# mauro3/KissMCMC.jl

Hardware: NVIDIA B200
Metric: walker_steps_per_s (higher is better)
Workload: dtype f64

## Files before the change

### kissmcmc.jl_b200/csrc/kmc_device.cuh

```cuda
#pragma once
#include <cstdint>
#ifndef KMC_U48_BITS
#define KMC_U48_BITS 0
#endif
#include <cuda_runtime.h>

namespace kmc {

__device__ __forceinline__ double dmul(double a, double b) { return __dmul_rn(a, b); }
__device__ __forceinline__ double dadd(double a, double b) { return __dadd_rn(a, b); }
__device__ __forceinline__ double dsub(double a, double b) { return __dsub_rn(a, b); }
__device__ __forceinline__ double ddiv(double a, double b) { return __ddiv_rn(a, b); }

__device__ __forceinline__ void split3_pair(double v0, double v1, unsigned (&pk)[3]) {
    float f0 = __double2float_rn(v0), f1 = __double2float_rn(v1);
#pragma unroll
    for (int pc = 0; pc < 3; ++pc) {
        unsigned u;
        asm("cvt.rn.bf16x2.f32 %0, %1, %2;" : "=r"(u) : "f"(f1), "f"(f0));
        pk[pc] = u;
        if (pc < 2) {
            f0 = __fsub_rn(f0, __uint_as_float(u << 16));
            f1 = __fsub_rn(f1, __uint_as_float(u & 0xFFFF0000u));
        }
    }
}

struct Philox4 {
    uint32_t r0, r1, r2, r3;
};

struct PhiloxKeys {
    uint32_t k0[10], k1[10];
};

__host__ __device__ inline PhiloxKeys philox_keys(uint64_t seed) {
    PhiloxKeys ks;
    uint32_t a = (uint32_t)seed, b = (uint32_t)(seed >> 32);
    for (int r = 0; r < 10; ++r) {
        ks.k0[r] = a;
        ks.k1[r] = b;
        a += 0x9E3779B9u;
        b += 0xBB67AE85u;
    }
    return ks;
}

__device__ __forceinline__ void mul_wide(uint32_t a, uint32_t b, uint32_t &hi, uint32_t &lo) {
    asm("{\n\t.reg .u64 t;\n\tmul.wide.u32 t, %2, %3;\n\tmov.b64 {%1, %0}, t;\n\t}" : "=r"(hi), "=r"(lo) : "r"(a), "r"(b));
}

__device__ __forceinline__ Philox4 philox4x32_10(uint32_t c0, uint32_t c1, uint32_t c2, uint32_t c3,
                                                 const PhiloxKeys &ks) {
#pragma unroll
    for (int r = 0; r < 10; ++r) {
        uint32_t hi0, lo0, hi1, lo1;
        mul_wide(0xD2511F53u, c0, hi0, lo0);
        mul_wide(0xCD9E8D57u, c2, hi1, lo1);
        c0 = hi1 ^ c1 ^ ks.k0[r];
        c1 = lo1;
        c2 = hi0 ^ c3 ^ ks.k1[r];
        c3 = lo0;
    }
    return Philox4{c0, c1, c2, c3};
}

__device__ __forceinline__ uint32_t lemire_retry(const PhiloxKeys &ks, uint32_t walker, uint32_t iter_lo,
                                              uint32_t iter_hi, uint32_t batch, uint32_t nhalf, uint32_t lemire_t) {
    uint32_t hi, lo, attempt = 0;
    do {
        ++attempt;
        const Philox4 rr = philox4x32_10(walker, iter_lo, iter_hi, batch | (attempt << 8), ks);
        mul_wide(rr.r0, nhalf, hi, lo);
    } while (lo < lemire_t);
    return hi;
}

__device__ __forceinline__ void draw(const PhiloxKeys &ks, uint32_t walker, uint32_t iter_lo, uint32_t iter_hi,
                                     uint32_t batch, uint32_t nhalf, uint32_t lemire_t, uint32_t &partner_local,
                                     double &uz, double &uacc) {
    const Philox4 r = philox4x32_10(walker, iter_lo, iter_hi, batch, ks);
    uint32_t hi, lo;
    mul_wide(r.r0, nhalf, hi, lo);
    if (lo < lemire_t)
        hi = lemire_retry(ks, walker, iter_lo, iter_hi, batch, nhalf, lemire_t);
    partner_local = hi;
    const uint64_t bz = ((uint64_t)r.r1 << 16) | (r.r2 >> 16);
    const uint64_t ba = ((uint64_t)(r.r2 & 0xFFFFu) << 32) | r.r3;
#if KMC_U48_BITS
    uz = __dadd_rn(__longlong_as_double((long long)(0x3FF0000000000000ULL | (bz << 4))), -1.0);
    uacc = __dadd_rn(__longlong_as_double((long long)(0x3FF0000000000000ULL | (ba << 4))), -1.0);
#else
    uz = (double)bz * 0x1p-48;
    uacc = (double)ba * 0x1p-48;
#endif
}

__device__ __forceinline__ Philox4 philox_normals(const PhiloxKeys &ks, uint32_t c0, uint32_t c1, uint32_t c2, uint32_t c3,
                                                  double &z0, double &z1) {
    const Philox4 r = philox4x32_10(c0, c1, c2, c3, ks);
    const double u1 = ((double)r.r0 + 1.0) * 0x1p-32;
    const double u2 = (double)r.r1 * 0x1p-32;
    const double rad = sqrt(-2.0 * log(u1));
    double sn, cs;
    sincospi(2.0 * u2, &sn, &cs);
    z0 = rad * cs;
    z1 = rad * sn;
    return r;
}


constexpr int KIND_EXPONENTIAL = 0;
constexpr int KIND_ROSENBROCK = 1;
constexpr int KIND_GAUSSIAN = 2;
constexpr int KIND_LOGNORMAL = 3;
constexpr int KIND_LOGISTIC = 4;

template <int D>
struct Exponential {
    static constexpr int kind = KIND_EXPONENTIAL;
    static constexpr int nparams = 0;
    double unused;
    __device__ __forceinline__ double logpdf(const double (&x)[D]) const {
        double s = x[0];
        bool neg = x[0] < 0.0;
#pragma unroll
        for (int c = 1; c < D; ++c) {
            neg = neg || (x[c] < 0.0);
            s = dadd(s, x[c]);
        }
        return neg ? -CUDART_INF : -s;
    }
};

__device__ __forceinline__ double ddiv_by(double a, double b, double y) {
    const double aa = fabs(a);
    if (y != 0.0 && aa > 0x1p-900 && aa < 0x1p900) {
        const double q0 = a * y;
        const double r0 = fma(-b, q0, a);
        const double q1 = fma(r0, y, q0);
        const double r1 = fma(-b, q1, a);
        return fma(r1, y, q1);
    }
    return __ddiv_rn(a, b);
}

template <int D>
struct Rosenbrock {
    static_assert(D == 2, "rosenbrock is 2-D");
    static constexpr int kind = KIND_ROSENBROCK;
    static constexpr int nparams = 3;
    double p[4];
    __device__ __forceinline__ double logpdf(const double (&x)[D]) const {
        const double t = dsub(x[1], dmul(x[0], x[0]));
        const double q = dmul(p[1], dmul(t, t));
        const double m = dsub(p[0], x[0]);
        const double r = dadd(q, dmul(m, m));
        return ddiv_by(-r, p[2], p[3]);
    }
};

template <int D>
struct Gaussian {
    static constexpr int kind = KIND_GAUSSIAN;
    static constexpr int nparams = D + D * D + 1;
    double p[D + D * D + 1];
    __device__ __forceinline__ double logpdf(const double (&x)[D]) const {
        double c[D];
#pragma unroll
        for (int j = 0; j < D; ++j) c[j] = dsub(x[j], p[j]);
        double ss = 0.0;
#pragma unroll
        for (int i = 0; i < D; ++i) {
            double y = 0.0;
#pragma unroll
            for (int j = 0; j < D; ++j) y = dadd(y, dmul(p[D + i * D + j], c[j]));
            ss = dadd(ss, dmul(y, y));
        }
        return dsub(p[D + D * D], dmul(0.5, ss));
    }
};

template <int D>
struct LogNormal {
    static_assert(D == 1, "lognormal is 1-D");
    static constexpr int kind = KIND_LOGNORMAL;
    static constexpr int nparams = 3;
    double p[3];
    __device__ __forceinline__ double logpdf(const double (&x)[D]) const {
        if (!(x[0] > 0.0)) return (x[0] != x[0]) ? x[0] : -CUDART_INF;
        const double lx = log(x[0]);
        const double t = ddiv(dsub(lx, p[0]), p[1]);
        return dsub(dsub(-lx, dmul(0.5, dmul(t, t))), p[2]);
    }
};

template <int D>
__device__ __forceinline__ void load_row(const double *__restrict__ p, double (&v)[D]) {
    if constexpr (D % 2 == 0) {
#pragma unroll
        for (int c = 0; c < D; c += 2) {
            const double2 t = *reinterpret_cast<const double2 *>(p + c);
            v[c] = t.x;
            v[c + 1] = t.y;
        }
    } else {
#pragma unroll
        for (int c = 0; c < D; ++c) v[c] = p[c];
    }
}

template <int D>
__device__ __forceinline__ void load_row_cg(const double *p, double (&v)[D]) {
    if constexpr (D % 2 == 0) {
#pragma unroll
        for (int c = 0; c < D; c += 2) {
            const double2 t = __ldcg(reinterpret_cast<const double2 *>(p + c));
            v[c] = t.x;
            v[c + 1] = t.y;
        }
    } else {
#pragma unroll
        for (int c = 0; c < D; ++c) v[c] = __ldcg(p + c);
    }
}

template <int D>
__device__ __forceinline__ void store_row(double *p, const double (&v)[D]) {
    if constexpr (D % 2 == 0) {
#pragma unroll
        for (int c = 0; c < D; c += 2) *reinterpret_cast<double2 *>(p + c) = make_double2(v[c], v[c + 1]);
    } else {
#pragma unroll
        for (int c = 0; c < D; ++c) p[c] = v[c];
    }
}

template <int D>
__device__ __forceinline__ void store_row_cs(double *p, const double (&v)[D]) {
    if constexpr (D % 2 == 0) {
#pragma unroll
        for (int c = 0; c < D; c += 2) __stcs(reinterpret_cast<double2 *>(p + c), make_double2(v[c], v[c + 1]));
    } else {
#pragma unroll
        for (int c = 0; c < D; ++c) __stcs(p + c, v[c]);
    }
}

}
```

### kissmcmc.jl_b200/csrc/kmc_kernels.cuh

```cuda
#pragma once
#include <math_constants.h>
#include <type_traits>

#include "kmc_device.cuh"

namespace kmc {

template <int D>
__host__ __device__ constexpr int max_threads() { return D <= 4 ? 448 : 256; }
template <int D>
__host__ __device__ constexpr int min_blocks() { return D <= 4 ? 2 : 1; }
template <int D>
__host__ __device__ constexpr int in_flight() { return D <= 2 ? 2 : (D <= 8 ? 2 : 1); }

struct RunParams {
    double *x;
    double *lp;
    unsigned *nacc;
    double *chain_x;
    double *chain_lp;
    const long long *rp_partner;
    const double *rp_z;
    const double *rp_u;
    long long rp_t0;
    long long nw;
    unsigned nhalf;
    unsigned per_cta;
    unsigned shard_begin, shard_end;
    long long chain_nw;
    long long h0, h1;
    long long n0;
    long long phase0;
    long long sidx0;
    long long nthin, ns;
    double sia, span, nm1;
    float nm1f, margin;
    PhiloxKeys keys;
    unsigned id_base[2];
    unsigned lemire_t;
    unsigned long long *barrier;
    unsigned long long bar_base;
    const double *peer_x[8];
    unsigned long long *peer_flags[8];
    int npeers, rank;
    unsigned long long epoch_base;
};

__device__ __forceinline__ void barrier_arrive(unsigned long long *ctr) {
    asm volatile("red.release.gpu.global.add.u64 [%0], 1;" ::"l"(ctr) : "memory");
}
__device__ __forceinline__ void barrier_wait(const unsigned long long *ctr, unsigned long long target) {
    unsigned long long v;
    long long t0 = 0;
    unsigned spins = 0;
    do {
        asm volatile("ld.relaxed.gpu.global.u64 %0, [%1];" : "=l"(v) : "l"(ctr) : "memory");
        if (v < target && (++spins & 0xFFFu) == 0) {
            if (t0 == 0) t0 = clock64();
            else if (clock64() - t0 > 40000000000LL) __trap();
        }
    } while (v < target);
    asm volatile("fence.acq_rel.gpu;" ::: "memory");
}

__device__ __forceinline__ void barrier_wait_acquire(const unsigned long long *ctr, unsigned long long target) {
    unsigned long long v;
    long long t0 = 0;
    unsigned spins = 0;
    do {
        asm volatile("ld.acquire.gpu.global.u64 %0, [%1];" : "=l"(v) : "l"(ctr) : "memory");
        if (v < target && (++spins & 0xFFFu) == 0) {
            if (t0 == 0) t0 = clock64();
            else if (clock64() - t0 > 40000000000LL) __trap();
        }
    } while (v < target);
}

template <bool SKIP_LOGZ>
__device__ __forceinline__ bool accept_exact(double nm1, double z, double p1, double p0, double u) {
    double lhs;
    if constexpr (SKIP_LOGZ) lhs = dsub(p1, p0);
    else lhs = dsub(dadd(dmul(nm1, log(z)), p1), p0);
    return lhs >= log(u);
}

__device__ __forceinline__ float lg2_approx(float v) {
    float r;
    asm("lg2.approx.ftz.f32 %0, %1;" : "=f"(r) : "f"(v));
    return r;
}

template <bool REPLAY>
__device__ __forceinline__ float filter_q(const RunParams &p, double z, double u) {
    const float zf = (float)z, uf = (float)u;
    bool ok = uf > 1e-30f;
    if constexpr (REPLAY) ok = ok && uf < 1e30f;
    ok = ok && zf > 0.0625f && zf < 16.0f;
    const float q = fmaf(p.nm1f, lg2_approx(zf), -lg2_approx(uf));
    return ok ? q : CUDART_NAN_F;
}

template <bool REPLAY>
__device__ __forceinline__ void step_draws(const RunParams &p, long long h, unsigned i, unsigned &j, double &z,
                                           double &u) {
    if constexpr (REPLAY) {
        const long long slot = (h - 2 * p.rp_t0) * (long long)p.nhalf + i;
        j = (unsigned)__ldcs(p.rp_partner + slot);
        z = __ldcs(p.rp_z + slot);
        u = __ldcs(p.rp_u + slot);
    } else {
        const unsigned long long t = (unsigned long long)(h >> 1);
        const unsigned batch = (unsigned)(h & 1);
        unsigned pl;
        double uz;
        draw(p.keys, p.id_base[batch] + i, (unsigned)t, (unsigned)(t >> 32), batch, p.nhalf, p.lemire_t, pl, uz, u);
        j = (batch ? 0u : p.nhalf) + pl;
        const double s = dadd(dmul(uz, p.span), p.sia);
        z = dmul(s, s);
    }
}

template <bool REPLAY, bool SKIP_LOGZ>
__device__ __forceinline__ bool accept_slow(const RunParams &p, long long h, unsigned i, double z, double p1, double p0) {
    unsigned j;
    double z2, u;
    step_draws<REPLAY>(p, h, i, j, z2, u);
    return accept_exact<SKIP_LOGZ>(p.nm1, z, p1, p0, u);
}

struct DrawRec {
    unsigned j;
    float q;
    double z;
};

__device__ __forceinline__ size_t chain_row(const RunParams &p, long long sidx, unsigned batch, unsigned i) {
    return (size_t)sidx * p.chain_nw + (batch ? (size_t)(p.shard_end - p.shard_begin) : 0) + (i - p.shard_begin);
}

template <int D>
__device__ __forceinline__ void chain_store(const RunParams &p, size_t o, bool acc, const double (&y)[D],
                                            const double (&xk)[D], double p1, double lpk) {
    if (acc) store_row_cs<D>(p.chain_x + o * D, y);
    else store_row_cs<D>(p.chain_x + o * D, xk);
    __stcs(p.chain_lp + o, acc ? p1 : lpk);
}

template <int D>
__device__ __forceinline__ void load_row_sys(const double *p, double (&v)[D]) {
    if constexpr (D % 2 == 0) {
#pragma unroll
        for (int c = 0; c < D; c += 2)
            asm volatile("ld.relaxed.sys.global.v2.f64 {%0, %1}, [%2];" : "=d"(v[c]), "=d"(v[c + 1]) : "l"(p + c) : "memory");
    } else {
#pragma unroll
        for (int c = 0; c < D; ++c) asm volatile("ld.relaxed.sys.global.f64 %0, [%1];" : "=d"(v[c]) : "l"(p + c) : "memory");
    }
}

__device__ __forceinline__ void bulk_row_g2s(void *smem_dst, const void *gsrc, unsigned bytes, unsigned long long *bar) {
    asm volatile("cp.async.bulk.shared::cluster.global.mbarrier::complete_tx::bytes [%0], [%1], %2, [%3];" ::"r"(
                     (unsigned)__cvta_generic_to_shared(smem_dst)),
                 "l"(gsrc), "r"(bytes), "r"((unsigned)__cvta_generic_to_shared(bar))
                 : "memory");
}
__device__ __forceinline__ void kbar_init(unsigned long long *bar, unsigned count) {
    asm volatile("mbarrier.init.shared::cta.b64 [%0], %1;" ::"r"((unsigned)__cvta_generic_to_shared(bar)), "r"(count));
    asm volatile("fence.mbarrier_init.release.cluster;" ::: "memory");
}
__device__ __forceinline__ void kbar_expect_tx(unsigned long long *bar, unsigned bytes) {
    asm volatile("mbarrier.arrive.expect_tx.shared::cta.b64 _, [%0], %1;" ::"r"((unsigned)__cvta_generic_to_shared(bar)),
                 "r"(bytes)
                 : "memory");
}
__device__ __forceinline__ void kbar_wait(unsigned long long *bar, unsigned parity) {
    const unsigned a = (unsigned)__cvta_generic_to_shared(bar);
    const long long t0 = clock64();
    unsigned done = 0;
    while (!done) {
        asm volatile(
            "{\n\t.reg .pred p;\n\t"
            "mbarrier.try_wait.parity.shared::cta.b64 p, [%1], %2;\n\t"
            "selp.u32 %0, 1, 0, p;\n\t}"
            : "=r"(done)
            : "r"(a), "r"(parity)
            : "memory");
        if (!done && clock64() - t0 > 20000000000LL) __trap();
    }
}

__device__ __forceinline__ void cross_gpu_barrier(const RunParams &p, unsigned long long epoch) {
    if ((int)threadIdx.x < p.npeers) {
        unsigned long long *dst = p.peer_flags[threadIdx.x] + p.rank;
        asm volatile("fence.acq_rel.sys;" ::: "memory");
        asm volatile("st.release.sys.global.u64 [%0], %1;" ::"l"(dst), "l"(epoch) : "memory");
        const unsigned long long *mine = p.peer_flags[p.rank] + threadIdx.x;
        const long long t0 = clock64();
        unsigned long long v;
        do {
            asm volatile("ld.acquire.sys.global.u64 %0, [%1];" : "=l"(v) : "l"(mine) : "memory");
            if (v < epoch && clock64() - t0 > 20000000000LL) __trap();
        } while (v < epoch);
    }
}

template <template <int> class Dn, int D, bool REPLAY, bool PEER = false>
static __global__ void __launch_bounds__(max_threads<D>(), min_blocks<D>()) emcee_run_kernel(const RunParams p,
                                                                                    const Dn<D> dn) {
    constexpr int U = in_flight<D>();
    const unsigned shard_size = p.shard_end - p.shard_begin;
    constexpr bool BULK = PEER && (D % 2 == 0);
    __shared__ __align__(16) double prow[BULK ? U * max_threads<D>() * D : 1];
    __shared__ unsigned long long pbar;
    unsigned pphase = 0;
    if constexpr (BULK) {
        if (threadIdx.x == 0) kbar_init(&pbar, 1);
        __syncthreads();
    }
    const unsigned tid = threadIdx.x, nthr = blockDim.x;
    const unsigned base = p.shard_begin + blockIdx.x * p.per_cta;
    const unsigned cnt = base >= p.shard_end ? 0u : min(p.per_cta, p.shard_end - base);

    DrawRec dr[U];
    auto make_draws = [&](long long h, unsigned l, DrawRec &r) {
        unsigned j;
        double z, u;
        step_draws<REPLAY>(p, h, base + l, j, z, u);
        r.j = j;
        r.z = z;
        r.q = filter_q<REPLAY>(p, z, u);
    };
#pragma unroll
    for (int q = 0; q < U; ++q) {
        const unsigned l = tid + q * nthr;
        if (l < cnt) make_draws(p.h0, l, dr[q]);
    }

    long long n = p.n0, phase = p.phase0, sidx = p.sidx0;
    unsigned long long target = p.bar_base;
    for (long long h = p.h0; h < p.h1; ++h) {
        const int batch = (int)(h & 1);
        const bool store = (n > 0) && (phase == 0);
        const unsigned a0 = batch ? p.nhalf : 0u;

        for (unsigned g = 0; g * nthr < cnt; g += U) {
            if (g > 0) {
#pragma unroll
                for (int q = 0; q < U; ++q) {
                    const unsigned l = tid + (g + q) * nthr;
                    if (l < cnt) make_draws(h, l, dr[q]);
                }
            }
            double xj[U][D], xk[U][D], lpk[U];
            if constexpr (BULK) {
                if (tid == 0) {
                    unsigned rows = 0;
#pragma unroll
                    for (int q = 0; q < U; ++q) {
                        const unsigned first = (g + q) * nthr;
                        rows += first < cnt ? min(nthr, cnt - first) : 0u;
                    }
                    kbar_expect_tx(&pbar, rows * D * 8);
                }
            }
#pragma unroll
            for (int q = 0; q < U; ++q) {
                const unsigned l = tid + (g + q) * nthr;
                if (l < cnt) {
                    const size_t k = (size_t)a0 + base + l;
                    if constexpr (PEER) {
                        const unsigned pos = dr[q].j >= p.nhalf ? dr[q].j - p.nhalf : dr[q].j;
                        const double *src = p.peer_x[pos / shard_size] + (size_t)dr[q].j * D;
                        if constexpr (BULK) bulk_row_g2s(prow + ((size_t)q * nthr + tid) * D, src, D * 8, &pbar);
                        else load_row_sys<D>(src, xj[q]);
                    } else {
                        load_row_cg<D>(p.x + (size_t)dr[q].j * D, xj[q]);
                    }
                    load_row<D>(p.x + k * D, xk[q]);
                    lpk[q] = p.lp[k];
                }
            }
            if constexpr (BULK) {
                kbar_wait(&pbar, pphase);
                pphase ^= 1;
#pragma unroll
                for (int q = 0; q < U; ++q) {
                    const unsigned l = tid + (g + q) * nthr;
                    if (l < cnt) {
#pragma unroll
                        for (int c = 0; c < D; ++c) xj[q][c] = prow[((size_t)q * nthr + tid) * D + c];
                    }
                }
                __syncthreads();
            }
#pragma unroll
            for (int q = 0; q < U; ++q) {
                const unsigned l = tid + (g + q) * nthr;
                if (l >= cnt) continue;
                const size_t k = (size_t)a0 + base + l;
                const double z = dr[q].z;
                double y[D];
#pragma unroll
                for (int c = 0; c < D; ++c) y[c] = dadd(xj[q][c], dmul(z, dsub(xk[q][c], xj[q][c])));
                const double p1 = dn.logpdf(y);
                const double tt = (p1 - lpk[q]) + (double)dr[q].q * 0.6931471805599453;
                bool acc;
                if (tt > (double)p.margin) acc = true;
                else if (tt < -(double)p.margin) acc = false;
                else acc = accept_slow<REPLAY, (D == 1 && !REPLAY)>(p, h, base + l, z, p1, lpk[q]);
                if (acc) {
                    store_row<D>(p.x + k * D, y);
                    p.lp[k] = p1;
                    p.nacc[k] += 1u;
                }
                if (store) chain_store<D>(p, chain_row(p, sidx, (unsigned)batch, base + l), acc, y, xk[q], p1, lpk[q]);
            }
        }
        if (batch == 1) {
            if (n == 0) {
                for (unsigned l = tid; l < cnt; l += nthr) {
                    p.nacc[base + l] = 0u;
                    p.nacc[(size_t)p.nhalf + base + l] = 0u;
                }
            }
            if (store) ++sidx;
            ++n;
            if (++phase == p.nthin) phase = 0;
        }
        if (h + 1 < p.h1) {
            target += gridDim.x;
            __syncthreads();
            if (gridDim.x > 1 && tid == 0) barrier_arrive(p.barrier);
#pragma unroll
            for (int q = 0; q < U; ++q) {
                const unsigned l = tid + q * nthr;
                if (l < cnt) make_draws(h + 1, l, dr[q]);
            }
            if (gridDim.x > 1) {
                if (tid == 0) barrier_wait(p.barrier, target);
                __syncthreads();
            }
            if constexpr (PEER) {
                if (blockIdx.x == 0) cross_gpu_barrier(p, p.epoch_base + (unsigned long long)(h - p.h0) + 1);
                target += gridDim.x;
                __syncthreads();
                if (gridDim.x > 1) {
                    if (tid == 0) {
                        barrier_arrive(p.barrier);
                        barrier_wait(p.barrier, target);
                    }
                    __syncthreads();
                }
            }
        }
    }
}

constexpr int kBulkThreads = 256;
#ifndef KMC_BULK_STORE_ALL
#define KMC_BULK_STORE_ALL 0
#endif
#ifndef KMC_BULK_CTAS
#define KMC_BULK_CTAS 3
#endif

__device__ __forceinline__ void bulk_s2g(void *gdst, const void *smem_src, unsigned bytes) {
    asm volatile("cp.async.bulk.global.shared::cta.bulk_group [%0], [%1], %2;" ::"l"(gdst),
                 "r"((unsigned)__cvta_generic_to_shared(smem_src)), "r"(bytes)
                 : "memory");
    asm volatile("cp.async.bulk.commit_group;" ::: "memory");
}

template <template <int> class Dn, int D, bool PEER>
static __global__ void __launch_bounds__(kBulkThreads, KMC_BULK_CTAS) emcee_bulk_kernel(const RunParams p, const Dn<D> dn) {
    static_assert(D % 2 == 0, "rows must be multiples of 16 bytes");
    extern __shared__ __align__(128) unsigned char bulk_smem[];
    constexpr unsigned T = kBulkThreads, ROWB = D * 8;
    double *xown = reinterpret_cast<double *>(bulk_smem);
    double *xpart = xown + 2 * T * D;
    unsigned long long *ldbar = reinterpret_cast<unsigned long long *>(xpart + T * D);
    const unsigned tid = threadIdx.x;
    const unsigned base = p.shard_begin + blockIdx.x * p.per_cta;
    const unsigned cnt = base >= p.shard_end ? 0u : min(p.per_cta, p.shard_end - base);
    const unsigned shard_size = p.shard_end - p.shard_begin;
    const unsigned ngroups = (cnt + T - 1) / T;
    if (tid == 0) kbar_init(ldbar, 1);
    __syncthreads();
    unsigned ldphase = 0, gcount = 0;

    DrawRec dr;
    auto make_draw = [&](long long h, unsigned l) {
        unsigned j;
        double z, u;
        step_draws<false>(p, h, base + l, j, z, u);
        dr.j = j;
        dr.z = z;
        dr.q = filter_q<false>(p, z, u);
    };
    if (tid < cnt) make_draw(p.h0, tid);

    long long n = p.n0, phase = p.phase0, sidx = p.sidx0;
    unsigned long long target = p.bar_base;
    for (long long h = p.h0; h < p.h1; ++h) {
        const unsigned batch = (unsigned)(h & 1);
        const bool store = (n > 0) && (phase == 0);
        const size_t a0 = batch ? (size_t)p.nhalf : 0;
        for (unsigned g = 0; g < ngroups; ++g, ++gcount) {
            const unsigned rows = min(T, cnt - g * T);
            const unsigned l = g * T + tid;
            const bool live = tid < rows;
            double *own = xown + (size_t)(gcount & 1) * T * D;
            if (tid == 0) asm volatile("cp.async.bulk.wait_group.read 1;" ::: "memory");
            __syncthreads();
            if (tid == 0) {
                kbar_expect_tx(ldbar, rows * ROWB * 2);
                bulk_row_g2s(own, p.x + (a0 + base + (size_t)g * T) * D, rows * ROWB, ldbar);
            }
            if (g > 0 && live) make_draw(h, l);
            if (live) {
                const unsigned pos = dr.j >= p.nhalf ? dr.j - p.nhalf : dr.j;
                const double *src = (PEER ? p.peer_x[pos / shard_size] : p.x) + (size_t)dr.j * D;
                bulk_row_g2s(xpart + (size_t)tid * D, src, ROWB, ldbar);
            }
            const size_t k = a0 + base + l;
            const double lpk = live ? p.lp[k] : 0.0;
            kbar_wait(ldbar, ldphase);
            ldphase ^= 1;
            if (live) {
                double xk[D], xj[D], y[D];
#pragma unroll
                for (int c = 0; c < D; c += 2) {
                    const double2 a2 = *reinterpret_cast<const double2 *>(own + (size_t)tid * D + c);
                    const double2 b2 = *reinterpret_cast<const double2 *>(xpart + (size_t)tid * D + c);
                    xk[c] = a2.x;
                    xk[c + 1] = a2.y;
                    xj[c] = b2.x;
                    xj[c + 1] = b2.y;
                }
                const double z = dr.z;
#pragma unroll
                for (int c = 0; c < D; ++c) y[c] = dadd(xj[c], dmul(z, dsub(xk[c], xj[c])));
                const double p1 = dn.logpdf(y);
                const double tt = (p1 - lpk) + (double)dr.q * 0.6931471805599453;
                bool acc;
                if (tt > (double)p.margin) acc = true;
                else if (tt < -(double)p.margin) acc = false;
                else acc = accept_slow<false, false>(p, h, base + l, z, p1, lpk);
                if (acc) {
#if KMC_BULK_STORE_ALL
#pragma unroll
                    for (int c = 0; c < D; c += 2)
                        *reinterpret_cast<double2 *>(own + (size_t)tid * D + c) = make_double2(y[c], y[c + 1]);
#else
                    store_row<D>(p.x + k * D, y);
#endif
                    p.lp[k] = p1;
                    p.nacc[k] += 1u;
                }
                if (store) chain_store<D>(p, chain_row(p, sidx, batch, base + l), acc, y, xk, p1, lpk);
            }
#if KMC_BULK_STORE_ALL
            asm volatile("fence.proxy.async.shared::cta;" ::: "memory");
            __syncthreads();
            if (tid == 0) bulk_s2g(p.x + (a0 + base + (size_t)g * T) * D, own, rows * ROWB);
#endif
        }
        if (batch == 1) {
            if (n == 0) {
                for (unsigned l = tid; l < cnt; l += T) {
                    p.nacc[base + l] = 0u;
                    p.nacc[(size_t)p.nhalf + base + l] = 0u;
                }
            }
            if (store) ++sidx;
            ++n;
            if (++phase == p.nthin) phase = 0;
        }
#if KMC_BULK_STORE_ALL
        if (tid == 0) {
            asm volatile("cp.async.bulk.wait_group 0;" ::: "memory");
            asm volatile("fence.proxy.async;" ::: "memory");
        }
#else
        asm volatile("fence.proxy.async;" ::: "memory");
#endif
        if (h + 1 < p.h1) {
            target += gridDim.x;
            __syncthreads();
            if (gridDim.x > 1 && tid == 0) barrier_arrive(p.barrier);
            if (tid < cnt) make_draw(h + 1, tid);
            if (gridDim.x > 1) {
                if (tid == 0) barrier_wait(p.barrier, target);
                __syncthreads();
            }
#if !KMC_BULK_STORE_ALL
            asm volatile("fence.proxy.async;" ::: "memory");
#endif
            if constexpr (PEER) {
                if (blockIdx.x == 0) cross_gpu_barrier(p, p.epoch_base + (unsigned long long)(h - p.h0) + 1);
                target += gridDim.x;
                __syncthreads();
                if (gridDim.x > 1) {
                    if (tid == 0) {
                        barrier_arrive(p.barrier);
                        barrier_wait(p.barrier, target);
                    }
                    __syncthreads();
                }
            }
        }
    }
}

#ifndef KMC_SMEM_ROUNDS
#define KMC_SMEM_ROUNDS 7
#endif
#ifndef KMC_SMEM_THREADS
#define KMC_SMEM_THREADS 256
#endif
#ifndef KMC_SMEM_CTAS
#define KMC_SMEM_CTAS 2
#endif
#ifndef KMC_SMEM_SPLIT
#define KMC_SMEM_SPLIT 4
#endif
constexpr int kRounds = KMC_SMEM_ROUNDS;
constexpr int kSmemSplit = KMC_SMEM_SPLIT;
#ifndef KMC_SMEM_AHEAD
#define KMC_SMEM_AHEAD 2
#endif
constexpr int kAhead = KMC_SMEM_AHEAD;
static_assert(kSmemSplit >= kAhead && kSmemSplit <= kRounds, "the first partner gathers need their draws");
constexpr int kSmemThreads = KMC_SMEM_THREADS;
constexpr int kSmemCtas = KMC_SMEM_CTAS;

__device__ __forceinline__ double lds_f64(unsigned a) {
    double v;
    asm volatile("ld.shared.f64 %0, [%1];" : "=d"(v) : "r"(a));
    return v;
}
__device__ __forceinline__ void sts_f64(unsigned a, double v) {
    asm volatile("st.shared.f64 [%0], %1;" ::"r"(a), "d"(v) : "memory");
}
__device__ __forceinline__ unsigned lds_u32(unsigned a) {
    unsigned v;
    asm volatile("ld.shared.u32 %0, [%1];" : "=r"(v) : "r"(a));
    return v;
}
__device__ __forceinline__ void sts_u32(unsigned a, unsigned v) {
    asm volatile("st.shared.u32 [%0], %1;" ::"r"(a), "r"(v) : "memory");
}

template <template <int> class Dn, int D, bool REPLAY>
static __global__ void __launch_bounds__(kSmemThreads, kSmemCtas) emcee_smem_kernel(const RunParams p, const Dn<D> dn) {
    extern __shared__ __align__(16) unsigned char smem_raw[];
    const unsigned nthr = blockDim.x;
    const unsigned L = 2 * p.per_cta;
    const unsigned wid = p.shard_begin + blockIdx.x * p.per_cta + threadIdx.x;
    const unsigned sbase = (unsigned)__cvta_generic_to_shared(smem_raw) + 8u * threadIdx.x;
    const unsigned nbase = (unsigned)__cvta_generic_to_shared(smem_raw) + 8u * (D + 1) * L + 4u * threadIdx.x;
    double *const grow = p.x + (size_t)wid * D;
    unsigned nv;
    {
        const unsigned base = p.shard_begin + blockIdx.x * p.per_cta;
        const unsigned cnt = base >= p.shard_end ? 0u : min(p.per_cta, p.shard_end - base);
        nv = cnt > threadIdx.x ? (cnt - threadIdx.x + nthr - 1) / nthr : 0u;
    }

    for (unsigned b = 0; b < 2; ++b)
        for (unsigned q = 0; q < nv; ++q) {
            const size_t ro = (size_t)b * p.nhalf + (size_t)q * nthr;
            const unsigned sl = b * p.per_cta + q * nthr;
            double v[D];
            load_row<D>(grow + ro * D, v);
#pragma unroll
            for (int c = 0; c < D; ++c) sts_f64(sbase + 8u * (c * L + sl), v[c]);
            sts_f64(sbase + 8u * (D * L + sl), p.lp[wid + ro]);
            sts_u32(nbase + 4u * sl, p.nacc[wid + ro]);
        }

    DrawRec dr[kRounds];
    auto make_draws = [&](long long h, auto lo, auto hi) {
#pragma unroll
        for (int q = decltype(lo)::value; q < decltype(hi)::value; ++q)
            if (q < nv) {
                unsigned j;
                double z, u;
                step_draws<REPLAY>(p, h, wid + q * nthr, j, z, u);
                dr[q].j = j;
                dr[q].z = z;
                dr[q].q = filter_q<REPLAY>(p, z, u);
            }
    };
    using SplitLo = std::integral_constant<int, 0>;
    using SplitMid = std::integral_constant<int, kSmemSplit>;
    using SplitHi = std::integral_constant<int, kRounds>;
    make_draws(p.h0, SplitLo{}, SplitMid{});

    const unsigned nh = (unsigned)(p.h1 - p.h0);
    long long n = p.n0;
    unsigned phase = (unsigned)p.phase0;
    long long sidx = p.sidx0;
    unsigned long long target = p.bar_base;
    for (unsigned hh = 0; hh < nh; ++hh) {
        const long long h = p.h0 + hh;
        const unsigned batch = (unsigned)(h & 1);
        const bool store = (n > 0) && (phase == 0);
        const unsigned hslot = batch ? p.per_cta : 0u;
        const size_t hrow = batch ? (size_t)p.nhalf : (size_t)0;

        double xj[kAhead][D];
#pragma unroll
        for (int q = 0; q < kAhead; ++q)
            if (q < nv) load_row_cg<D>(p.x + (size_t)dr[q].j * D, xj[q]);
        make_draws(h, SplitMid{}, SplitHi{});
#pragma unroll
        for (int q = 0; q < kRounds; ++q) {
            if (q >= nv) break;
            const unsigned sl = hslot + q * nthr;
            const size_t ro = hrow + (size_t)q * nthr;
            double xk[D], y[D];
#pragma unroll
            for (int c = 0; c < D; ++c) xk[c] = lds_f64(sbase + 8u * (c * L + sl));
            const double lpk = lds_f64(sbase + 8u * (D * L + sl));
            const double z = dr[q].z;
#pragma unroll
            for (int c = 0; c < D; ++c) y[c] = dadd(xj[q % kAhead][c], dmul(z, dsub(xk[c], xj[q % kAhead][c])));
            if (q + kAhead < kRounds && q + kAhead < nv)
                load_row_cg<D>(p.x + (size_t)dr[(q + kAhead) % kRounds].j * D, xj[q % kAhead]);
            const double p1 = dn.logpdf(y);
            const double tt = (p1 - lpk) + (double)dr[q].q * 0.6931471805599453;
            bool acc;
            if (tt > (double)p.margin) acc = true;
            else if (tt < -(double)p.margin) acc = false;
            else acc = accept_slow<REPLAY, (D == 1 && !REPLAY)>(p, h, wid + q * nthr, z, p1, lpk);
            if (acc) {
                store_row<D>(grow + ro * D, y);
#pragma unroll
                for (int c = 0; c < D; ++c) sts_f64(sbase + 8u * (c * L + sl), y[c]);
                sts_f64(sbase + 8u * (D * L + sl), p1);
                sts_u32(nbase + 4u * sl, lds_u32(nbase + 4u * sl) + 1u);
            }
            if (store) chain_store<D>(p, chain_row(p, sidx, batch, wid + q * nthr), acc, y, xk, p1, lpk);
        }
        if (batch == 1) {
            if (n == 0)
                for (unsigned q = 0; q < nv; ++q) {
                    sts_u32(nbase + 4u * (q * nthr), 0u);
                    sts_u32(nbase + 4u * (p.per_cta + q * nthr), 0u);
                }
            if (store) ++sidx;
            ++n;
            if (++phase == (unsigned)p.nthin) phase = 0;
        }
        if (hh + 1 < nh) {
            target += gridDim.x;
            __syncthreads();
            if (gridDim.x > 1 && threadIdx.x == 0) barrier_arrive(p.barrier);
            make_draws(h + 1, SplitLo{}, SplitMid{});
            if (gridDim.x > 1) {
                if (threadIdx.x == blockDim.x - 32) barrier_wait_acquire(p.barrier, target);
                __syncthreads();
            }
        }
    }

    for (unsigned b = 0; b < 2; ++b)
        for (unsigned q = 0; q < nv; ++q) {
            const size_t ro = (size_t)b * p.nhalf + (size_t)q * nthr;
            const unsigned sl = b * p.per_cta + q * nthr;
            p.lp[wid + ro] = lds_f64(sbase + 8u * (D * L + sl));
            p.nacc[wid + ro] = lds_u32(nbase + 4u * sl);
        }
}

template <template <int> class Dn, int D>
static __global__ void __launch_bounds__(256) density_eval_kernel(const double *__restrict__ x, double *__restrict__ out,
                                                           long long nw, const Dn<D> dn) {
    const long long w = (long long)blockIdx.x * blockDim.x + threadIdx.x;
    if (w >= nw) return;
    double v[D];
    load_row<D>(x + w * D, v);
    out[w] = dn.logpdf(v);
}

constexpr long long kTransposeMaxSamples = 65535LL * 32;
static __global__ void chain_transpose_kernel(const double *__restrict__ in, double *__restrict__ out, long long ns,
                                       long long nw, long long w0, long long wc, int d, long long s0) {
    __shared__ double tile[32][33];
    const int c = blockIdx.z;
    const long long wb = (long long)blockIdx.x * 32, sb = s0 + (long long)blockIdx.y * 32;
    for (int r = threadIdx.y; r < 32; r += blockDim.y) {
        const long long s = sb + r, w = wb + threadIdx.x;
        if (s < ns && w < wc) tile[r][threadIdx.x] = in[(s * nw + (w0 + w)) * d + c];
    }
    __syncthreads();
    for (int r = threadIdx.y; r < 32; r += blockDim.y) {
        const long long w = wb + r, s = sb + threadIdx.x;
        if (s < ns && w < wc) out[(w * ns + s) * d + c] = tile[threadIdx.x][r];
    }
}

static __global__ void __launch_bounds__(256) chain_moments_kernel(const double *__restrict__ chain, long long nrows, int d,
                                                            double *__restrict__ sums ) {
    extern __shared__ double sh[];
    for (int c = threadIdx.x; c < 2 * d; c += blockDim.x) sh[c] = 0.0;
    __syncthreads();
    const long long total = nrows * d;
    for (long long e = (long long)blockIdx.x * blockDim.x + threadIdx.x; e < total; e += (long long)gridDim.x * blockDim.x) {
        const int c = (int)(e % d);
        const double v = chain[e] - chain[c];
        atomicAdd(&sh[c], v);
        atomicAdd(&sh[d + c], v * v);
    }
    __syncthreads();
    for (int c = threadIdx.x; c < 2 * d; c += blockDim.x) atomicAdd(&sums[c], sh[c]);
}

static __global__ void nacc_sum_kernel(const unsigned *__restrict__ nacc, long long nw, unsigned long long *sum) {
    unsigned long long s = 0;
    for (long long i = (long long)blockIdx.x * blockDim.x + threadIdx.x; i < nw; i += (long long)gridDim.x * blockDim.x)
        s += nacc[i];
    for (int o = 16; o > 0; o >>= 1) s += __shfl_xor_sync(0xffffffffu, s, o);
    if ((threadIdx.x & 31) == 0 && s) atomicAdd(sum, s);
}

static __global__ void nacc_moment_kernel(const unsigned *__restrict__ nacc, long long nw, double mean, double thresh,
                                   double *ssq, unsigned long long *outl) {
    double s = 0.0;
    unsigned long long o = 0;
    for (long long i = (long long)blockIdx.x * blockDim.x + threadIdx.x; i < nw; i += (long long)gridDim.x * blockDim.x) {
        const double dv = (double)nacc[i] - mean;
        s += dv * dv;
        o += (thresh >= 0.0 && fabs(dv) > thresh) ? 1 : 0;
    }
    for (int k = 16; k > 0; k >>= 1) {
        s += __shfl_xor_sync(0xffffffffu, s, k);
        o += __shfl_xor_sync(0xffffffffu, o, k);
    }
    if ((threadIdx.x & 31) == 0) {
        if (ssq) atomicAdd(ssq, s);
        if (outl && o) atomicAdd(outl, o);
    }
}

}
```

Before: 88.52 billion.

## Defer Rosenbrock division refinement and batch undecided accepts into a cold loop

Splits the Rosenbrock logpdf so the accept/reject test uses only the cheap reciprocal-multiply estimate, widening the margin by a relative bound, and runs the Newton refinement only for decided walkers. Walkers whose decision falls in the margin band are collected in a bitmask and handled afterwards in a separate non-unrolled loop that redraws their randoms, recomputes the proposal and applies the exact accept test. The aim is to cut divergent slow-path work and FMA count out of the hot unrolled loop. It costs recomputation for undecided walkers and relies on accept_exact and step_draws helpers matching the old accept_slow semantics.

```diff
diff --git a/kissmcmc.jl_b200/csrc/kmc_device.cuh b/kissmcmc.jl_b200/csrc/kmc_device.cuh
--- a/kissmcmc.jl_b200/csrc/kmc_device.cuh
+++ b/kissmcmc.jl_b200/csrc/kmc_device.cuh
@@ -133,15 +133,19 @@
     }
 };
 
+__device__ __forceinline__ bool ddiv_by_in_range(double a, double y) {
+    const double aa = fabs(a);
+    return y != 0.0 && aa > 0x1p-900 && aa < 0x1p900;
+}
+__device__ __forceinline__ double ddiv_by_refine(double a, double b, double y, double q0) {
+    const double r0 = fma(-b, q0, a);
+    const double q1 = fma(r0, y, q0);
+    const double r1 = fma(-b, q1, a);
+    return fma(r1, y, q1);
+}
 __device__ __forceinline__ double ddiv_by(double a, double b, double y) {
     const double aa = fabs(a);
-    if (y != 0.0 && aa > 0x1p-900 && aa < 0x1p900) {
-        const double q0 = a * y;
-        const double r0 = fma(-b, q0, a);
-        const double q1 = fma(r0, y, q0);
-        const double r1 = fma(-b, q1, a);
-        return fma(r1, y, q1);
-    }
+    if (y != 0.0 && aa > 0x1p-900 && aa < 0x1p900) return ddiv_by_refine(a, b, y, a * y);
     return __ddiv_rn(a, b);
 }
 
@@ -151,12 +155,34 @@
     static constexpr int kind = KIND_ROSENBROCK;
     static constexpr int nparams = 3;
     double p[4];
-    __device__ __forceinline__ double logpdf(const double (&x)[D]) const {
+    __device__ __forceinline__ double numerator(const double (&x)[D]) const {
         const double t = dsub(x[1], dmul(x[0], x[0]));
         const double q = dmul(p[1], dmul(t, t));
         const double m = dsub(p[0], x[0]);
         const double r = dadd(q, dmul(m, m));
-        return ddiv_by(-r, p[2], p[3]);
+        return -r;
+    }
+    __device__ __forceinline__ double logpdf(const double (&x)[D]) const { return ddiv_by(numerator(x), p[2], p[3]); }
+};
+
+template <template <int> class Dn, int D>
+struct LogpdfSplit {
+    static constexpr double kRel = 0.0;
+};
+
+template <int D>
+struct LogpdfSplit<Rosenbrock, D> {
+    static constexpr double kRel = 0x1p-50;
+    double a, q0;
+    bool ok;
+    __device__ __forceinline__ double decide(const Rosenbrock<D> &dn, const double (&x)[D]) {
+        a = dn.numerator(x);
+        q0 = dmul(a, dn.p[3]);
+        ok = ddiv_by_in_range(a, dn.p[3]);
+        return q0;
+    }
+    __device__ __forceinline__ double finish(const Rosenbrock<D> &dn) const {
+        return ok ? ddiv_by_refine(a, dn.p[2], dn.p[3], q0) : __ddiv_rn(a, dn.p[2]);
     }
 };
 
diff --git a/kissmcmc.jl_b200/csrc/kmc_kernels.cuh b/kissmcmc.jl_b200/csrc/kmc_kernels.cuh
--- a/kissmcmc.jl_b200/csrc/kmc_kernels.cuh
+++ b/kissmcmc.jl_b200/csrc/kmc_kernels.cuh
@@ -614,11 +614,23 @@
         for (int q = 0; q < kAhead; ++q)
             if (q < nv) load_row_cg<D>(p.x + (size_t)dr[q].j * D, xj[q]);
         make_draws(h, SplitMid{}, SplitHi{});
+        auto commit = [&](int q, bool acc, const double (&y)[D], const double (&xk)[D], double p1, double lpk) {
+            const unsigned sl = hslot + q * nthr;
+            const size_t ro = hrow + (size_t)q * nthr;
+            if (acc) {
+                store_row<D>(grow + ro * D, y);
+#pragma unroll
+                for (int c = 0; c < D; ++c) sts_f64(sbase + 8u * (c * L + sl), y[c]);
+                sts_f64(sbase + 8u * (D * L + sl), p1);
+                sts_u32(nbase + 4u * sl, lds_u32(nbase + 4u * sl) + 1u);
+            }
+            if (store) chain_store<D>(p, chain_row(p, sidx, batch, wid + q * nthr), acc, y, xk, p1, lpk);
+        };
+        unsigned undecided = 0;
 #pragma unroll
         for (int q = 0; q < kRounds; ++q) {
             if (q >= nv) break;
             const unsigned sl = hslot + q * nthr;
-            const size_t ro = hrow + (size_t)q * nthr;
             double xk[D], y[D];
 #pragma unroll
             for (int c = 0; c < D; ++c) xk[c] = lds_f64(sbase + 8u * (c * L + sl));
@@ -628,20 +640,44 @@
             for (int c = 0; c < D; ++c) y[c] = dadd(xj[q % kAhead][c], dmul(z, dsub(xk[c], xj[q % kAhead][c])));
             if (q + kAhead < kRounds && q + kAhead < nv)
                 load_row_cg<D>(p.x + (size_t)dr[(q + kAhead) % kRounds].j * D, xj[q % kAhead]);
+            using Split = LogpdfSplit<Dn, D>;
+            constexpr bool kSplit = Split::kRel != 0.0;
+            Split lp1;
+            double p1;
+            if constexpr (kSplit) p1 = lp1.decide(dn, y);
+            else p1 = dn.logpdf(y);
+            const double tt = (p1 - lpk) + (double)dr[q].q * 0.6931471805599453;
+            double thr = (double)p.margin;
+            bool fast = true;
+            if constexpr (kSplit) {
+                thr = fma(fabs(p1), Split::kRel, thr);
+                fast = lp1.ok;
+            }
+            const bool acc = fast && tt > thr;
+            const bool decided = acc || (fast && tt < -thr);
+            if (decided) {
+                if constexpr (kSplit) p1 = lp1.finish(dn);
+                commit(q, acc, y, xk, p1, lpk);
+            } else {
+                undecided |= 1u << q;
+            }
+        }
+#pragma unroll 1
+        for (unsigned rest = undecided; rest; rest &= rest - 1) {
+            const unsigned q = __ffs(rest) - 1;
+            const unsigned sl = hslot + q * nthr;
+            unsigned j;
+            double z, u;
+            step_draws<REPLAY>(p, h, wid + q * nthr, j, z, u);
+            double xk[D], xjq[D], y[D];
+#pragma unroll
+            for (int c = 0; c < D; ++c) xk[c] = lds_f64(sbase + 8u * (c * L + sl));
+            const double lpk = lds_f64(sbase + 8u * (D * L + sl));
+            load_row_cg<D>(p.x + (size_t)j * D, xjq);
+#pragma unroll
+            for (int c = 0; c < D; ++c) y[c] = dadd(xjq[c], dmul(z, dsub(xk[c], xjq[c])));
             const double p1 = dn.logpdf(y);
-            const double tt = (p1 - lpk) + (double)dr[q].q * 0.6931471805599453;
-            bool acc;
-            if (tt > (double)p.margin) acc = true;
-            else if (tt < -(double)p.margin) acc = false;
-            else acc = accept_slow<REPLAY, (D == 1 && !REPLAY)>(p, h, wid + q * nthr, z, p1, lpk);
-            if (acc) {
-                store_row<D>(grow + ro * D, y);
-#pragma unroll
-                for (int c = 0; c < D; ++c) sts_f64(sbase + 8u * (c * L + sl), y[c]);
-                sts_f64(sbase + 8u * (D * L + sl), p1);
-                sts_u32(nbase + 4u * sl, lds_u32(nbase + 4u * sl) + 1u);
-            }
-            if (store) chain_store<D>(p, chain_row(p, sidx, batch, wid + q * nthr), acc, y, xk, p1, lpk);
+            commit((int)q, accept_exact<(D == 1 && !REPLAY)>(p.nm1, z, p1, lpk, u), y, xk, p1, lpk);
         }
         if (batch == 1) {
             if (n == 0)
```

Measured after the change: 83.50 billion, median of 6. 5.7% lower.
